# D-Robotics/hobot_stereonet

Measured on AMD Instinct MI355X. Metric: stereo pairs/s at 1280x720 D=192 (ms/frame alongside), higher is better.
Workload: dtype f16 (refinement-tower MFMA operands fp16 — 3x3 weights rounded per kernel so that every kernel's tap sum survives —, LeakyReLU applied after the fp16 rounding; low-resolution branch on 22-bit hi/lo split fp16 operands, 3 fp16 MFMAs per product in every 32-channel layer — profiles/r04_lowres_ablation

## Files before the change

hobot_stereonet_amd/csrc/sn_dbg_hooks.hpp:

```cpp
#pragma once

namespace {

void host_to_slots(const float* src, int nimg, int H, int W, std::vector<_Float16>& dst) {
  const size_t plane = (size_t)H * W;
  dst.assign((size_t)nimg * 8 * plane * 8, (_Float16)0.f);
  for (int img = 0; img < nimg; ++img)
    for (int c = 0; c < kC; ++c)
      for (size_t i = 0; i < plane; ++i) {
        const float v = src[((size_t)img * kC + c) * plane + i];
        const _Float16 hi = (_Float16)v;
        const size_t base = (((size_t)img * 4 + (c >> 3)) * 2) * plane;
        dst[(base + i) * 8 + (c & 7)] = hi;
        dst[(base + plane + i) * 8 + (c & 7)] = (_Float16)((v - (float)hi) * kSplitScale);
      }
}
void host_from_slots(const std::vector<_Float16>& src, int nimg, int H, int W, float* dst) {
  const size_t plane = (size_t)H * W;
  for (int img = 0; img < nimg; ++img)
    for (int c = 0; c < kC; ++c)
      for (size_t i = 0; i < plane; ++i) {
        const size_t base = (((size_t)img * 4 + (c >> 3)) * 2) * plane;
        dst[((size_t)img * kC + c) * plane + i] =
            (float)src[(base + i) * 8 + (c & 7)] + (float)src[(base + plane + i) * 8 + (c & 7)] * kSplitInv;
// ... 236 lines not shown
  for (size_t i = 0; i < be.size(); ++i) beff[i] = (float)be[i];
  return SN_OK;
}

int sn_dbg_down01(sn_handle* h, const int8_t* in6, int h_px, int w, const float* w0, const float* b0, const float* w1,
                  const float* b1, float* out) {
  DevScope ds;
  if (!h || !in6 || !w0 || !b0 || !w1 || !b1 || !out || h_px <= 0 || w <= 0) return SN_ERR_ARG;
  int rc = check_device(h);
  if (rc) return rc;
  const int Hp = (h_px + 15) / 16 * 16, Wp = (w + 15) / 16 * 16, Ho = Hp / 4, Wo = Wp / 4;
  Down01W L;
  rc = upload_down01(h, HostLayer{w0, b0, kC, 3, 25}, HostLayer{w1, b1, kC, kC, 25}, &L);
  ds.adopt(L);
  if (rc) return rc;
  int8_t* din = nullptr;
  uint4* dout = nullptr;
  const size_t nin = (size_t)6 * h_px * w, nout = (size_t)2 * kC * Ho * Wo;
  HIP_TRY(h, ds.alloc(&din, nin));
  HIP_TRY(h, ds.alloc(&dout, nout / 4));
  HIP_TRY(h, hipMemcpy(din, in6, nin, hipMemcpyHostToDevice));
  HIP_TRY(h, launch_down01(h->stream, L, din, h_px, w, 2, Ho, Wo, dout, SlotGeom{Ho, Wo, 0, 0}, h->num_cu));
  HIP_TRY(h, hipStreamSynchronize(h->stream));
  std::vector<_Float16> hs(nout * 2);
  HIP_TRY(h, from_dev(hs, dout));
  host_from_slots(hs, 2, Ho, Wo, out);
  return SN_OK;
}

int sn_dbg_refin(sn_handle* h, const float* disp_low, const int8_t* in6, int h_px, int w, int dmax, const float* wt,
                 const float* bias, int split, float* out) {
  DevScope ds;
  if (!h || !disp_low || !in6 || !wt || !bias || !out || h_px <= 0 || w <= 0 || dmax <= 0) return SN_ERR_ARG;
  int rc = check_device(h);
  if (rc) return rc;
  const int Hp = (h_px + 15) / 16 * 16, Wp = (w + 15) / 16 * 16, hl = Hp / 16, wl = Wp / 16;
  RefHost t(make_ref_geom(Hp, Wp), 1, Hp, Wp, true, true);
  Down0F16 L;
  rc = upload_refin_f16(h, HostLayer{wt, bias, kC, 4, 9}, &L);
  ds.adopt(L);
  if (rc) return rc;
  float *ddl = nullptr, *dbias = nullptr;
  int8_t* din = nullptr;
  uint4* dout = nullptr;
  HIP_TRY(h, ds.alloc(&ddl, (size_t)hl * wl));
  HIP_TRY(h, ds.alloc(&dbias, kC));
  HIP_TRY(h, ds.alloc(&din, (size_t)6 * h_px * w));
  HIP_TRY(h, ds.alloc(&dout, t.slots()));
  HIP_TRY(h, hipMemcpy(ddl, disp_low, (size_t)hl * wl * 4, hipMemcpyHostToDevice));
  HIP_TRY(h, hipMemcpy(dbias, bias, kC * 4, hipMemcpyHostToDevice));
  HIP_TRY(h, hipMemcpy(din, in6, (size_t)6 * h_px * w, hipMemcpyHostToDevice));
  HIP_TRY(h, memset_now(dout, 0, t.slots() * 16));
  HIP_TRY(h, launch_refin_f16(h->stream, L, dbias, ddl, din, false, hl, wl, h_px, w, 1.0f / (float)dmax,
                              UpScale{1.0f / 16.0f, 16.0f}, t.g, 1, dout, split != 0, t.lo_slots * 16, h->num_cu));
  HIP_TRY(h, hipStreamSynchronize(h->stream));
  HIP_TRY(h, from_dev(t.v, dout));
  t.unpack(out, split != 0);
  if (!t.border_is_zero(1)) {
    set_err(h, "ref.in wrote into the zero border");
    return SN_ERR_DEVICE;
  }
  return SN_OK;
}

int sn_dbg_conv3d(sn_handle* h, const float* in, int d, int h_px, int w, const float* wt, const float* bias,
                  int lrelu, float* out) {
  DevScope ds;
  if (!h || !in || !wt || !bias || !out || d <= 0) return SN_ERR_ARG;
  int rc = check_device(h);
  if (rc) return rc;
  const bool x3 = (lrelu & 2) != 0, slots = (lrelu & 4) != 0, dma = (lrelu & 8) != 0;
  lrelu &= 1;
  if (slots != x3 || (dma && !slots)) return SN_ERR_ARG;
  ConvLayer L;
  rc = upload_conv3d(h, HostLayer{wt, bias, kC, kC, 27}, &L);
  if (!rc && x3)
    rc = upload_x3(h, 96, [&](int co, int c, int tap) { return wt[(((size_t)co * kC + (c & 31)) * 3 + (c >> 5)) * 9 + tap]; }, &L);
  ds.adopt(L);
  if (rc) return rc;
  const size_t plane = (size_t)h_px * w, n = (size_t)kC * d * plane;
  std::vector<float> tmp(n);
  for (int ci = 0; ci < kC; ++ci)
    for (int z = 0; z < d; ++z)
      memcpy(&tmp[((size_t)z * kC + ci) * plane], &in[((size_t)ci * d + z) * plane], plane * 4);
  float *din = nullptr, *dout = nullptr;
  HIP_TRY(h, ds.alloc(&din, n));
  HIP_TRY(h, ds.alloc(&dout, n));
  if (slots) {
    std::vector<_Float16> hs, ho(n * 2);
    host_to_slots(tmp.data(), d, h_px, w, hs);
    if (dma) {
      const VolPad g = vol_pad(d, h_px, w);
      PaddedSlots pin(SlotGeom{g.PH, g.PW, 1, 1}, h_px, w, (size_t)d * 8, 8), pout = pin;
      pin.put(hs);
      uint4 *pdin = nullptr, *pdout = nullptr;
      HIP_TRY(h, ds.alloc(&pdin, pin.v.size() / 8));
      HIP_TRY(h, ds.alloc(&pdout, pout.v.size() / 8));
      HIP_TRY(h, to_dev(pdin, pin.v));
      HIP_TRY(h, memset_now(pdout, 0, pout.v.size() * 2));
      HIP_TRY(h, launch_agg_dma<true>(h->stream, L, pdin, g, 1, pdout, lrelu != 0, h->num_cu));
      HIP_TRY(h, hipStreamSynchronize(h->stream));
      HIP_TRY(h, from_dev(pout.v, pdout));
      pout.get(ho);
      if (!pout.outside_is_zero()) {
        set_err(h, "k_agg_x3s_dma wrote outside the image");
        return SN_ERR_DEVICE;
      }
// ... 294 lines not shown
```

hobot_stereonet_amd/csrc/sn_engine.hpp:

```cpp
#pragma once

namespace {

using namespace sn;

constexpr int kNDown = 4, kNFeatRes = 6, kNAgg = 4, kNRefRes = 6;
constexpr int kRefDil[kNRefRes] = {1, 2, 4, 8, 1, 1};
constexpr float kOutScale = 2.60443857769133e-6f;
constexpr double kWireFactor = 16.0 * 12.0;
constexpr double kAutoEnvelopeSingle = 1.0, kAutoEnvelopeMulti = 2.9;
constexpr double kAutoResidualCap = 1e30;
constexpr int kMaxPieceEvents = 64;
constexpr int kMaxTowerStreams = 2;

#define HIP_TRY(h, expr)                                                              \
  do {                                                                                \
    hipError_t e_ = (expr);                                                           \
    if (e_ != hipSuccess) {                                                           \
      set_err(h, std::string(#expr) + ": " + hipGetErrorString(e_));                  \
      return SN_ERR_DEVICE;                                                           \
    }                                                                                 \
  } while (0)

inline hipError_t memset_now(void* p, int v, size_t bytes) {
// ... 123 lines not shown
  hipStream_t stream = nullptr;
  hipEvent_t ev0 = nullptr, ev1 = nullptr;
  Workspace ws;
  int8_t* pin_in = nullptr;
  int32_t* pin_raw = nullptr;
  float* pin_disp = nullptr;
  int32_t* user_raw = nullptr;
  float* user_disp = nullptr;
  uint64_t ticket = 0;
  hipGraphExec_t gexec[2][4][4] = {};
  int uses[2][4][4] = {};
  int mode_run = 0;
};

struct RangeCount {
  unsigned long long level[4] = {}, low = 0;
  bool any() const { return (level[0] | level[1] | level[2] | level[3] | low) != 0; }
};

struct AutoCtl {
  sn_auto_state st{};
  bool calibrated = false;
  bool pending = false;
  int pending_mode = 0, pending_n = 0;
  double selfcheck_epe = -1.0, selfcheck_res = -1.0;
  double last_level[4] = {}, last_res = 0.0;
  RangeCount last_range;
  int last_mode = 0;
  uint64_t calls = 0, pairs = 0, reruns = 0;
};

}

struct sn_handle {
  int device = 0;
  int W = 0, H = 0, D = 0, Wp = 0, Hp = 0, wl = 0, hl = 0, Dl = 0;
  int max_batch = 1, precision = SN_PREC_F16, task_num = 4, refine_chunk = 1, piece = 16;
  AutoCtl actl;
  std::mutex mu_cal;
  float* chk[2] = {nullptr, nullptr};
  hipEvent_t ev_stats = nullptr;
  int refine_chunk_x3 = 1;
  hipStream_t stream = nullptr;
  hipStream_t s_low = nullptr, s_tow[kMaxTowerStreams] = {};
  hipEvent_t ev_fork = nullptr, ev_join = nullptr, ev_tow_join[kMaxTowerStreams] = {}, ev_piece[kMaxPieceEvents] = {};
  bool overlap = true;
  int tower_streams = kMaxTowerStreams;
#if SN_DIAGNOSTICS
  unsigned ablate_x = 0;
#else
  static constexpr unsigned ablate_x = 0;
#endif
  bool obstacle_rle = true;
  bool tail_fuse = true;
  int fuse_mode = 4;
  unsigned* dump = nullptr;
  bool use_graphs = true;
  bool stream_prio = false;
  ConvLayer down[kNDown], fres[kNFeatRes][2], fout, agg[kNAgg];
  Down0F16 down0;
  Down01W down01;
  bool fold_down01 = false;
  HeadLayer aout;
  int levels = 1;
  Tower tw[kMaxLevels];
  int num_cu = 256;
  Workspace ws;
  std::vector<Slot> slots;
  std::mutex mu;
  std::condition_variable cv;
  uint64_t next_ticket = 1;
  bool profiling = false;
  hipEvent_t ev[8] = {};
  hipEvent_t ev_dom[2 * 6] = {};
  int dom_pairs = 0;
  float stage_ms[SN_STAGE_COUNT] = {};
  mutable std::string err;
  mutable std::mutex err_mu;
  struct PointCloudSlots {
    enum { kScratch = 0, kRaw, kNv12, kPoints, kCounts, kPinRaw, kPinNv12, kCount };
  };
  struct PointCloud : Lane<PointCloudSlots> {
    PointCloud() { buf[kPinRaw].pinned = buf[kPinNv12].pinned = true; }
  } pc;
  struct FilterSlots {
    enum { kScratch = 0, kRaw, kDisp, kMask, kCounts, kCount };
  };
  using Filter = Lane<FilterSlots>;
  Filter flt;
  struct SmoothSlots {
    enum { kScratch = 0, kRaw, kGuide, kOut, kDisp, kMask, kCounts, kCount };
  };
  using Smooth = Lane<SmoothSlots>;
  Smooth smo;
  struct JpegSlots {
    enum { kCoef = 0, kBytes, kLens, kIn, kOut, kSizes, kCount };
  };
  struct Jpeg : Lane<JpegSlots> {
    sn::JpgPlan plan;
  } jpg;
  struct RenderSlots {
    enum { kRaw = 0, kLeft, kOut, kCanvas, kCoef, kBytes, kLens, kJpegOut, kSizes, kCount };
  };
  struct Render : Lane<RenderSlots> {
    sn::JpgPlan plan;
  } rnd;
// ... 82 lines not shown
```

hobot_stereonet_amd/csrc/sn_forward.hpp:

```cpp
#pragma once

namespace {

inline int piece_pairs(const sn_handle* h, int nb, int rb) {
  int pb = h->piece > 0 ? h->piece : 16;
  if (pb > nb) pb = nb;
  if (pb < rb) pb = rb;
  return pb;
}
inline int level_chunk_pairs(int rb, int pb, int lv) {
  const long r = (long)rb << (2 * lv);
  return lv == 0 ? rb : (r < pb ? (int)r : pb);
}

int alloc_ws(sn_handle* h, Workspace* ws, int nb, int rb, int ns, int rb_x3 = 0) {
  const bool is_auto = h->precision == SN_PREC_AUTO;
  if (rb_x3 <= 0 || rb_x3 > rb) rb_x3 = rb;
  ws->nb = nb;
  ws->rb = rb;
  ws->rb_x3 = rb_x3;
  ws->ns = (ns > 1 && nb > rb) ? (ns < kMaxTowerStreams ? ns : kMaxTowerStreams) : 1;
  if (h->levels > 1) ws->ns = 1;
  ws->pb = piece_pairs(h, nb, rb);
  const int pb = ws->pb;
// ... 290 lines not shown
  float dnorm;
  float* od;
  int32_t* orw;
  unsigned* chunk_ctr;
  int c;
  int cap;
  bool pe;
  int mode;
  unsigned long long* stat;
};

int refine_level(sn_handle* h, Workspace& ws, hipStream_t st, const RefineCall& a) {
  const Tower& T = *a.T;
  const int ncu = h->num_cu, c = a.c;
  const int tcu = ws.tower_cu > 0 ? ws.tower_cu : ncu;
  const int Hk = T.Hk, Wk = T.Wk;
  const bool pe = a.pe;
  const float inv_q = (float)(1.0 / (kWireFactor * (double)kOutScale));
  if (a.mode == SN_PREC_FP32) {
    LoadRefineIn ld{a.src, reinterpret_cast<const int8_t*>(a.img_src), a.sh, a.sw, a.H, a.W, Hk, Wk, 1.0f / a.dnorm, a.ups,
                    a.pyr ? reinterpret_cast<const float*>(a.img_src) : nullptr};
    if (Hk * Wk <= 64 * 128)
      HIP_TRY(h, (launch_conv<3, 1, 1, 4, 4, 32>(st, T.rin, ld, c, Hk, Wk, a.ref[0], nullptr, true)));
    else
      HIP_TRY(h, (launch_conv<3, 1, 1, 4, 8, 64>(st, T.rin, ld, c, Hk, Wk, a.ref[0], nullptr, true)));
    if (pe) HIP_TRY(h, hipEventRecord(h->ev[4], st));
    for (int i = 0; i < kNRefRes; ++i) {
      HIP_TRY(h, conv3x3(st, T.rres[i][0], a.ref[0], c, Hk, Wk, kRefDil[i], a.ref[1], nullptr, true, ncu));
      HIP_TRY(h, conv3x3(st, T.rres[i][1], a.ref[1], c, Hk, Wk, kRefDil[i], a.ref[0], a.ref[0], true, ncu));
    }
    if (pe) HIP_TRY(h, hipEventRecord(h->ev[5], st));
    const HeadArgs ha{T.rout.w, a.src, a.od, a.orw, T.rout.bias, a.dnorm, inv_q, a.sh, a.sw, a.H, a.W, a.ups, a.stat};
    if (switches().head_mfma32) {
      constexpr int TH = 14;
      using HT = HeadTile<TH>;
      const int tiles_x = (a.W + HT::TWO - 1) / HT::TWO, tiles_y = (a.H + TH - 1) / TH;
      hipLaunchKernelGGL(k_head_final_mfma32<TH>, dim3((unsigned)(tiles_x * tiles_y * c)), dim3(256), HT::LDS_BYTES, st, a.ref[0],
                         Hk, Wk, tiles_x, tiles_y, ha);
    } else {
      dim3 grid((a.W + 63) / 64, (a.H + 3) / 4, c);
      hipLaunchKernelGGL(k_head_final, grid, dim3(256), 0, st, a.ref[0], Hk, Wk, ha);
    }
  } else {
    uint4 *x16 = a.ref16[0], *t16 = a.ref16[1];
    if (pe) h->dom_pairs = 0;
    const bool rev_env = switches().rev;
    RefGeom g = T.rg;
    int launch_no = 0;
    auto flip = [&]() { g.rev = rev_env ? (launch_no++ & 1) : 0; };
    flip();
    const bool x3 = a.mode == SN_PREC_F16X3;
    const size_t lo_slots = ref16_slots(g, a.cap) + ref_slack(g);
    HIP_TRY(h, launch_refin_f16(st, T.refin, T.rin.bias, a.src, a.img_src, a.pyr, a.sh, a.sw, a.H, a.W, 1.0f / a.dnorm, a.ups, g,
                                c, x16, x3, lo_slots * 16, ncu));
    if (pe) HIP_TRY(h, hipEventRecord(h->ev[4], st));
    flip();
    const HeadArgs ha{T.rout.wsplit, a.src, a.od, a.orw, T.rout.biassplit, a.dnorm * T.rout.unscale, inv_q, a.sh, a.sw,
                      a.H, a.W, a.ups, a.stat};
    const bool last_streamed = h->fuse_mode == 4 && stream_block_supports(kRefDil[kNRefRes - 1]);
    const bool tail = !x3 && last_streamed && h->tail_fuse && kRefDil[kNRefRes - 1] == 1 && a.ups.rs <= 0.5f;
    for (int i = 0; i < kNRefRes; ++i) {
      if (x3) {
        const bool dom = pe && stream_x3_supports(kRefDil[i]) && h->dom_pairs < 6;
        if (dom) HIP_TRY(h, hipEventRecord(h->ev_dom[2 * h->dom_pairs], st));
        HIP_TRY(h, ref_block_f16x3(st, T.rres16x3[i][0], T.rres16x3[i][1], g, tcu, kRefDil[i], &x16, &t16, lo_slots, c));
        if (dom) HIP_TRY(h, hipEventRecord(h->ev_dom[2 * h->dom_pairs++ + 1], st));
      } else if (tail && i == kNRefRes - 1) {
        if (pe) HIP_TRY(h, hipEventRecord(h->ev[5], st));
        HIP_TRY(h, ref_block_stream_tail(st, T.rres16[i][0], T.rres16[i][1], g, tcu, x16, c, h->dump, ha));
      } else {
        const bool dom = pe && h->fuse_mode == 4 && stream_block_supports(kRefDil[i]) && h->dom_pairs < 6;
        if (dom) HIP_TRY(h, hipEventRecord(h->ev_dom[2 * h->dom_pairs], st));
        HIP_TRY(h, ref_block_f16(st, T.rres16[i][0], T.rres16[i][1], g, tcu, kRefDil[i], &x16, &t16, c,
                                 a.chunk_ctr + 2 * i * kTileCtrStride, h->fuse_mode, h->dump, rev_env));
        if (dom) HIP_TRY(h, hipEventRecord(h->ev_dom[2 * h->dom_pairs++ + 1], st));
      }
    }
    if (!tail) {
      if (pe) HIP_TRY(h, hipEventRecord(h->ev[5], st));
      HIP_TRY(h, launch_head_final_f16(st, x3, x16, lo_slots, g, c, ha));
    }
  }
  HIP_TRY(h, hipGetLastError());
  return SN_OK;
}

inline int chunk_pairs(const sn_handle* h, const Workspace& ws, int mode, int lv = 0) {
  return (h->precision == SN_PREC_AUTO && mode == SN_PREC_F16X3) ? ws.rbk_x3[lv] : ws.rbk[lv];
}

inline int take_ctr_block(sn_handle* h, Workspace& ws, int* ctr_block, unsigned** out) {
  *out = nullptr;
  if (!ws.tile_ctr) return SN_OK;
  if (*ctr_block >= ws.n_chunks) {
    set_err(h, "internal: tile-queue pool exhausted");
    return SN_ERR_DEVICE;
  }
  *out = ws.tile_ctr + (size_t)(*ctr_block)++ * (kTileCtrBytes / sizeof(unsigned));
  return SN_OK;
}

int refine_coarse(sn_handle* h, Workspace& ws, hipStream_t st, int p0, int m, const int8_t* in6, int* ctr_block, int mode) {
  const size_t HW = (size_t)h->H * h->W;
  const int8_t* in_piece = in6 + (size_t)p0 * 6 * HW;
  for (int lv = 1; lv < h->levels; ++lv) {
    const Tower& T = h->tw[lv];
    const long total = (long)m * 3 * T.Hk * T.Wk;
// ... 342 lines not shown
```

hobot_stereonet_amd/csrc/sn_kernels.hpp:

```cpp
#pragma once
#include <hip/hip_runtime.h>
#include <stdint.h>

#include <type_traits>

#ifndef SN_X3S_FPK
#define SN_X3S_FPK 2
#endif
#ifndef SN_X3S_WAGPR
#define SN_X3S_WAGPR 1
#endif

namespace sn {

typedef float f32x16 __attribute__((ext_vector_type(16)));
typedef float f32x4 __attribute__((ext_vector_type(4)));

typedef _Float16 half8 __attribute__((ext_vector_type(8)));
typedef _Float16 half4 __attribute__((ext_vector_type(4)));

constexpr int kC = 32;
constexpr int kRefPad = 8;
constexpr float kSplitScale = 2048.0f;
constexpr float kSplitInv = 1.0f / 2048.0f;
// ... 1561 lines not shown
#pragma unroll
      for (int i = 0; i < 2 * T::NSTORE; ++i) asm volatile("" : "+v"(rres[i]));
    }
    const bool interior = y0 + T::TH <= g.H && x0 + T::TW <= g.W;
#pragma unroll
    for (int q = 0; q < 4; ++q) {
      char* oq = reinterpret_cast<char*>(out) + (tb + (unsigned)q * plane_b);
      char* oql = out_lo + (tb + (unsigned)q * plane_b);
#pragma unroll
      for (int s = 0; s < T::SPW; ++s) {
        half4 hh, hl;
#pragma unroll
        for (int e = 0; e < 4; ++e) {
          float v = acc0[s][4 * q + e] + acc1[s][4 * q + e] * kSplitInv;
          if (RES) {
            const uint2 rh = rres[RES ? 2 * (s * 4 + q) : 0], rl = rres[RES ? 2 * (s * 4 + q) + 1 : 0];
            const half4 vh = *reinterpret_cast<const half4*>(&rh);
            const half4 vl = *reinterpret_cast<const half4*>(&rl);
            v += (float)vh[e] + (float)vl[e] * kSplitInv;
          }
          if (lrelu) v = lrelu_fast(v);
          const _Float16 hi = (_Float16)v;
          hh[e] = hi;
          hl[e] = (_Float16)((v - (float)hi) * kSplitScale);
        }
        if (!interior) {
          const int seg = seg0 + s;
          const int y = y0 + seg / T::CSEG, x = x0 + (seg % T::CSEG) * 32 + j;
          if (!(y < g.H && x < g.W)) {
            hh = half4{(_Float16)0.f, (_Float16)0.f, (_Float16)0.f, (_Float16)0.f};
            hl = hh;
          }
        }
        *reinterpret_cast<half4*>(oq + io_voff[s]) = hh;
        *reinterpret_cast<half4*>(oql + io_voff[s]) = hl;
      }
    }
    img = nimg_;
    y0 = ny0;
    x0 = nx0;
  }
}

template <int TW_>
struct RefInTile {
  static constexpr int TH = 8, TW = TW_, CSEG = TW / 32;
  static constexpr int ROWS = TH + 2, COLS = TW + 8;
  static constexpr int BUF = ROWS * COLS;
  static constexpr int LDS_BYTES = 2 * BUF * 16;
  static constexpr int NUNIT = ROWS * (COLS / 4);
  static constexpr int SPW = TH * CSEG / 4;
};

template <bool SPLIT, bool PYR, int TW>
__global__ __launch_bounds__(256, 2) void k_refin_f16(const float* __restrict__ disp_low,
                                                   const void* __restrict__ img_src,
                                                   int hl, int wl, int H, int W, float inv_d, UpScale ups,
                                                   const uint4* __restrict__ wfrag,
                                                   const float* __restrict__ bias, uint4* __restrict__ out,
                                                   size_t lo_off_bytes, RefGeom g, int nimg, int al4) {
  using T = RefInTile<TW>;
  static_assert(T::NUNIT <= 256, "one staging unit per thread");
  extern __shared__ __attribute__((aligned(16))) uint4 s_px[];
  const int tid = threadIdx.x, lane = tid & 63;
  const int wave = __builtin_amdgcn_readfirstlane(tid >> 6);
  const int j = lane & 31, gk = lane >> 5;

  half8 wa[5], wb[5];
#pragma unroll
  for (int t = 0; t < 5; ++t) {
    const uint4 a = wfrag[(2 * t) * 64 + lane], b = wfrag[(2 * t + 1) * 64 + lane];
    wa[t] = *reinterpret_cast<const half8*>(&a);
    wb[t] = *reinterpret_cast<const half8*>(&b);
  }
  f32x16 bv;
#pragma unroll
  for (int r = 0; r < 16; ++r) bv[r] = bias[(r & 3) + 8 * (r >> 2) + 4 * gk];
  int koff[5];
#pragma unroll
  for (int t = 0; t < 5; ++t) {
    int tap = 2 * t + gk;
    tap = tap < 9 ? tap : 0;
    koff[t] = (tap / 3) * T::COLS + (tap % 3) + 3;
  }

  const int per_img = g.tiles_x * g.tiles_y;
  const int total = per_img * nimg;
  const int ur = tid / (T::COLS / 4), uq = tid - ur * (T::COLS / 4);
  const bool unit = tid < T::NUNIT;
  const int8_t* const in6 = reinterpret_cast<const int8_t*>(img_src);
  const float* const pyr = reinterpret_cast<const float*>(img_src);
  const bool x16 = ups.rs == 1.0f / 16.0f;
  uint32_t pimg[3];
  float pf[PYR ? 3 : 1][4];
  float pd[4];
  bool pval[4];
  auto fetch = [&](int tile) {
    if (g.rev) tile = total - 1 - tile;
    const int img = tile / per_img, rem = tile - img * per_img;
    const int ty = rem / g.tiles_x, tx = rem - ty * g.tiles_x;
    const int y = ty * T::TH - 1 + ur, x = tx * T::TW - 4 + 4 * uq;
    pimg[0] = pimg[1] = pimg[2] = 0;
#pragma unroll
    for (int k = 0; k < 4; ++k) {
      pd[k] = 0.f;
      pval[k] = false;
    }
    if (!unit || (unsigned)y >= (unsigned)g.H) return;
    const float* dl = disp_low + (size_t)img * hl * wl;
#pragma unroll
    for (int k = 0; k < 4; ++k) pval[k] = (unsigned)(x + k) < (unsigned)g.W;
    if (x16 && x >= 0) {
      float sy = ((float)y + 0.5f) * ups.rs - 0.5f;
      sy = sy < 0.f ? 0.f : sy;
      float sx0 = ((float)x + 0.5f) * ups.rs - 0.5f;
// ... 23 lines not shown
        for (int k = 0; k < 4; ++k) pf[PYR ? c : 0][k] = pval[k] ? row[x + k] : 0.f;
      }
    } else if (y < H) {
#pragma unroll
      for (int c = 0; c < 3; ++c) {
        const int8_t* row = in6 + (((size_t)img * 6 + c) * H + y) * (size_t)W;
        uint32_t v = 0;
        if (al4) {
          if (x >= 0 && x + 3 < W) v = *reinterpret_cast<const uint32_t*>(row + x);
        } else {
#pragma unroll
          for (int k = 0; k < 4; ++k)
            if ((unsigned)(x + k) < (unsigned)W) v |= (uint32_t)(uint8_t)row[x + k] << (8 * k);
        }
        pimg[c] = v;
      }
    }
  };
  auto commit = [&](uint4* buf) {
    if (!unit) return;
#pragma unroll
    for (int k = 0; k < 4; ++k) {
      half8 sl;
#pragma unroll
      for (int e = 0; e < 8; ++e) sl[e] = (_Float16)0.f;
      if (pval[k]) {
        const _Float16 dh = (_Float16)pd[k];
        sl[0] = dh;
        sl[4] = (_Float16)((pd[k] - (float)dh) * kSplitScale);
        if (PYR) {
#pragma unroll
          for (int c = 0; c < 3; ++c) {
            const float v = pf[PYR ? c : 0][k];
            const _Float16 vh = (_Float16)v;
            sl[1 + c] = vh;
            sl[5 + c] = (_Float16)((v - (float)vh) * kSplitScale);
          }
        } else {
#pragma unroll
          for (int c = 0; c < 3; ++c) sl[1 + c] = (_Float16)((float)(int8_t)(pimg[c] >> (8 * k)) * (1.0f / 128.0f));
        }
      }
      buf[ur * T::COLS + 4 * uq + k] = *reinterpret_cast<const uint4*>(&sl);
    }
  };

  int tile = blockIdx.x;
  if (tile >= total) return;
  fetch(tile);
  commit(s_px);
  __syncthreads();
  int cur = 0;
  const unsigned plane_b = (unsigned)g.Hs * (unsigned)g.Ws * 16u;
  unsigned io_voff[T::SPW];
#pragma unroll
  for (int s = 0; s < T::SPW; ++s) {
    const int seg = wave * T::SPW + s;
    io_voff[s] = ((unsigned)(seg / T::CSEG) * (unsigned)g.Ws + (unsigned)((seg % T::CSEG) * 32 + j)) * 16u + gk * 8u;
  }
  for (; tile < total; tile += gridDim.x) {
    const int nxt = tile + gridDim.x;
    if (nxt < total) fetch(nxt);
    const uint4* buf = s_px + cur * T::BUF;
    f32x16 acc0[T::SPW], acc1[T::SPW];
    f32x16 zero;
#pragma unroll
    for (int r = 0; r < 16; ++r) zero[r] = 0.f;
#pragma unroll
    for (int t = 0; t < 5; ++t) {
#pragma unroll
      for (int s = 0; s < T::SPW; ++s) {
        const int seg = wave * T::SPW + s;
        const int srow = seg / T::CSEG, scol = (seg % T::CSEG) * 32;
        const uint4 xv = buf[koff[t] + srow * T::COLS + scol + j];
        const half8 xb = *reinterpret_cast<const half8*>(&xv);
        acc0[s] = __builtin_amdgcn_mfma_f32_32x32x16_f16(wa[t], xb, t == 0 ? bv : acc0[s], 0, 0, 0);
        acc1[s] = __builtin_amdgcn_mfma_f32_32x32x16_f16(wb[t], xb, t == 0 ? zero : acc1[s], 0, 0, 0);
      }
    }
    {
      const int tile_m = g.rev ? total - 1 - tile : tile;
      const int img = tile_m / per_img, rem = tile_m - img * per_img;
      const int ty = rem / g.tiles_x, tx = rem - ty * g.tiles_x;
      const int y0 = ty * T::TH, x0 = tx * T::TW;
      const bool interior = y0 + T::TH <= g.H && x0 + T::TW <= g.W;
      const unsigned tb = (((unsigned)img * 4u * (unsigned)g.Hs + (unsigned)(y0 + kRefPad)) * (unsigned)g.Ws +
                           (unsigned)(x0 + kRefPad)) * 16u;
#pragma unroll
      for (int s = 0; s < T::SPW; ++s) {
#pragma unroll
        for (int q = 0; q < 4; ++q) {
          char* oq = reinterpret_cast<char*>(out) + (tb + (unsigned)q * plane_b);
          char* oql = oq + lo_off_bytes;
          half4 hh, hl4;
          if (SPLIT) {
#pragma unroll
            for (int e = 0; e < 4; ++e) {
              float v = acc0[s][4 * q + e] + acc1[s][4 * q + e] * kSplitInv;
              v = lrelu_fast(v);
              const _Float16 hi = (_Float16)v;
              hh[e] = hi;
              hl4[e] = (_Float16)((v - (float)hi) * kSplitScale);
            }
          } else {
            float v[4];
#pragma unroll
            for (int e = 0; e < 4; ++e) v[e] = acc0[s][4 * q + e] + acc1[s][4 * q + e] * kSplitInv;
            const uint2 pk{act_pack2_f16(v[0], v[1], (_Float16)kSlope), act_pack2_f16(v[2], v[3], (_Float16)kSlope)};
            hh = *reinterpret_cast<const half4*>(&pk);
          }
          bool ok = true;
          if (!interior) {
            const int seg = wave * T::SPW + s;
            ok = y0 + seg / T::CSEG < g.H && x0 + (seg % T::CSEG) * 32 + j < g.W;
          }
          if (ok) {
            *reinterpret_cast<half4*>(oq + io_voff[s]) = hh;
            if (SPLIT) *reinterpret_cast<half4*>(oql + io_voff[s]) = hl4;
          }
        }
      }
    }
    if (nxt < total) commit(s_px + (cur ^ 1) * T::BUF);
    lds_barrier();
    cur ^= 1;
  }
}

template <int TH_>
struct HeadTile {
  static constexpr int TH = TH_, TWO = 62;
  static constexpr int RP = TH + 2, CP = 64;
  static constexpr int NSEG = RP * 2, SPW = (NSEG + 3) / 4;
  static constexpr int PLANE = RP * CP;
  static constexpr int LDS_BYTES = 9 * PLANE * 4;
};

template <int TH>
__device__ __forceinline__ void head_window_finish(const float* s_p, int n, int y0, int x0, const HeadArgs& ha) {
  using T = HeadTile<TH>;
  const float* dl = ha.disp_low + (size_t)n * ha.hl * ha.wl;
  float moved = 0.f;
  unsigned bad = 0u;
  for (int p = threadIdx.x; p < T::TH * T::TWO; p += 256) {
    const int oy = p / T::TWO, ox = p - oy * T::TWO;
    const int y = y0 + oy, x = x0 + ox;
    if (y >= ha.H || x >= ha.W) continue;
    float acc = ha.bias;
#pragma unroll
    for (int ky = 0; ky < 3; ++ky)
#pragma unroll
      for (int kx = 0; kx < 3; ++kx) acc += s_p[(ky * 3 + kx) * T::PLANE + (oy + ky) * T::CP + ox + kx];
    float mv;
    unsigned nf;
    const float d = head_value(upsample_map(dl, ha.hl, ha.wl, y, x, ha.ups), ha.dmax, acc, mv, nf);
    moved += mv;
    bad += nf;
    head_store(ha.out_disp, ha.out_raw, ((size_t)n * ha.H + y) * ha.W + x, d, ha.inv_q);
  }
  refine_stat_commit_block(ha.stat, moved, bad);
}

template <bool SPLIT, int TH>
__global__ __launch_bounds__(256) void k_head_final_f16(const uint4* __restrict__ xin, size_t lo_slots, RefGeom g,
                                                        int tiles_x, int tiles_y, HeadArgs ha) {
  using T = HeadTile<TH>;
  extern __shared__ __attribute__((aligned(16))) float s_p[];
  const int tid = threadIdx.x, lane = tid & 63;
  const int wave = __builtin_amdgcn_readfirstlane(tid >> 6);
  const int j = lane & 31, gh = lane >> 5;
  int t = blockIdx.x;
  const int tx = t % tiles_x;
  t /= tiles_x;
  const int ty = t % tiles_y, n = t / tiles_y;
  const int y0 = ty * T::TH, x0 = tx * T::TWO;

// ... 118 lines not shown
```

hobot_stereonet_amd/csrc/sn_launch.hpp:

```cpp
#pragma once

namespace {

template <class K>
hipError_t ensure_lds_attr(K kern, int bytes) {
  static std::mutex mu;
  static std::unordered_map<const void*, unsigned long long> done;
  int dev = 0;
  if (hipGetDevice(&dev) != hipSuccess) dev = 0;
  const unsigned long long bit = 1ull << (dev & 63);
  const void* key = reinterpret_cast<const void*>(kern);
  std::lock_guard<std::mutex> lk(mu);
  unsigned long long& m = done[key];
  if (m & bit) return hipSuccess;
  const hipError_t e = hipFuncSetAttribute(key, hipFuncAttributeMaxDynamicSharedMemorySize, bytes);
  if (e == hipSuccess) m |= bit;
  return e;
}

inline ConvArgs make_conv_args(const ConvLayer& L, const void* w, void* out, const void* res, int nimg, int Ho, int Wo, int dil,
                               int pad, bool lrelu, int TR, int TC) {
  ConvArgs a{};
  a.wpk = reinterpret_cast<const float*>(w);
  a.bias = L.bias;
  a.out = reinterpret_cast<float*>(out);
  a.res = reinterpret_cast<const float*>(res);
  a.nimg = nimg;
  a.cin_pad = L.cin_pad;
  a.Ho = Ho;
  a.Wo = Wo;
  a.dil = dil;
  a.pad = pad;
  a.lrelu = lrelu ? 1 : 0;
  a.tiles_x = (Wo + TC - 1) / TC;
  a.tiles_y = (Ho + TR - 1) / TR;
  return a;
}

inline int xcd_band_grid(int cap, int total) {
  const int need = (total + 7) / 8 * 8;
  return ((cap > need ? need : cap) + 7) / 8 * 8;
}

template <int TW>
hipError_t launch_refin_f16_tw(hipStream_t st, const Down0F16& L, const float* bias, const float* disp_low,
                               const void* img_src, bool pyr, int hl, int wl, int H, int W, float inv_d, UpScale ups,
                               RefGeom g, int nimg, uint4* out, bool split, size_t lo_off_bytes, int num_cu) {
  using T = RefInTile<TW>;
  g.tiles_x = (g.W + TW - 1) / TW;
  g.tiles_y = (g.H + T::TH - 1) / T::TH;
  const int total = g.tiles_x * g.tiles_y * nimg;
  int blocks = 2 * num_cu;
  if (blocks > total) blocks = total;
  const int al4 = !pyr && (W % 4 == 0) && (reinterpret_cast<uintptr_t>(img_src) % 4 == 0);
#define SN_REFIN(S, P)                                                                                             \
  hipLaunchKernelGGL((k_refin_f16<S, P, TW>), dim3(blocks), dim3(256), T::LDS_BYTES, st, disp_low, img_src, hl, wl, H, \
                     W, inv_d, ups, L.wfrag, bias, out, lo_off_bytes, g, nimg, al4)
  if (split && pyr) SN_REFIN(true, true);
  else if (split) SN_REFIN(true, false);
  else if (pyr) SN_REFIN(false, true);
  else SN_REFIN(false, false);
#undef SN_REFIN
  return hipGetLastError();
}

hipError_t launch_refin_f16(hipStream_t st, const Down0F16& L, const float* bias, const float* disp_low,
                            const void* img_src, bool pyr, int hl, int wl, int H, int W, float inv_d, UpScale ups,
                            const RefGeom& g, int nimg, uint4* out, bool split, size_t lo_off_bytes, int num_cu) {
  return launch_refin_f16_tw<64>(st, L, bias, disp_low, img_src, pyr, hl, wl, H, W, inv_d, ups, g, nimg, out, split,
                                 lo_off_bytes, num_cu);
}

hipError_t launch_down0_f16(hipStream_t st, const Down0F16& L, const float* bias, const int8_t* in6, int H, int W,
                            int nimg, int Ho, int Wo, float* out, int num_cu, const SlotGeom* og = nullptr) {
  constexpr int TC = 32;
  using T = Down0Tile<TC>;
  const int tiles_x = (Wo + TC - 1) / TC, tiles_y = (Ho + T::TR - 1) / T::TR;
  const int total = tiles_x * tiles_y * nimg;
  int blocks = 2 * num_cu;
  if (blocks > total) blocks = total;
  const int al4 = (W % 4 == 0) && (reinterpret_cast<uintptr_t>(in6) % 4 == 0);
  hipLaunchKernelGGL((k_down0_f16<TC>), dim3(blocks), dim3(256), T::LDS_BYTES, st, in6, H, W, L.wfrag, bias, out, Ho, Wo,
                     tiles_x, tiles_y, nimg, 0, al4, og ? og->PH : Ho, og ? og->PW : Wo, og ? og->py : 0, og ? og->px : 0);
  return hipGetLastError();
}

template <bool W4>
hipError_t launch_down01_w(hipStream_t st, const Down01W& L, const int8_t* in6, int H, int W, int nimg, int Ho, int Wo,
                           uint4* out, const SlotGeom& og, int num_cu) {
  using T = Down01;
  hipError_t e = ensure_lds_attr(k_down01_f16<W4>, T::LDS_BYTES);
  if (e != hipSuccess) return e;
  const int tiles_x = (Wo + T::TC - 1) / T::TC, tiles_y = (Ho + T::TR - 1) / T::TR;
  const int total = tiles_x * tiles_y * nimg;
  int blocks = num_cu / 8 * 8;
  while (blocks > 8 && blocks / 8 > (total + 7) / 8) blocks -= 8;
  hipLaunchKernelGGL(k_down01_f16<W4>, dim3(blocks), dim3(256), T::LDS_BYTES, st, in6, H, W,
                     L.wfrag + (size_t)T::INNER * T::NK * 2 * 64, L.bias + T::INNER * kC, out, Ho, Wo, tiles_x, tiles_y, nimg,
                     og.PH, og.PW, og.py, og.px);
  const int per_img = 4 + 2 * ((Wo - 2 + 31) / 32) + 2 * ((Ho - 2 + 31) / 32);
  hipLaunchKernelGGL(k_down01_border<W4>, dim3(per_img * (nimg / 2)), dim3(192), 0, st, in6, H, W, L.wfrag, L.bias, out,
                     Ho, Wo, nimg, og.PH, og.PW, og.py, og.px);
  return hipGetLastError();
}
hipError_t launch_down01(hipStream_t st, const Down01W& L, const int8_t* in6, int H, int W, int nimg, int Ho, int Wo,
                         uint4* out, const SlotGeom& og, int num_cu) {
  return (W % 4) == 0 ? launch_down01_w<true>(st, L, in6, H, W, nimg, Ho, Wo, out, og, num_cu)
                      : launch_down01_w<false>(st, L, in6, H, W, nimg, Ho, Wo, out, og, num_cu);
}

template <int KS, int STRIDE, int VCH, int TR, int TC, int SEGW, int MINB, bool OUTSLOT, class Loader, bool HASRES = false>
hipError_t launch_conv_x3s(hipStream_t st, const ConvLayer& L, const Loader& ld, int nimg, int Ho, int Wo, float* out,
                           const float* res, bool lrelu, int num_cu) {
  using T = X3sTile<KS, STRIDE, VCH, TR, TC, SEGW>;
  const ConvArgs a = make_conv_args(L, L.wx3, out, res, nimg, Ho, Wo, 1, KS / 2, lrelu, TR, TC);
  if (res != nullptr && !HASRES)
    return launch_conv_x3s<KS, STRIDE, VCH, TR, TC, SEGW, MINB, OUTSLOT, Loader, true>(st, L, ld, nimg, Ho, Wo, out, res, lrelu, num_cu);
  auto kern = k_conv_x3s<KS, STRIDE, VCH, TR, TC, SEGW, MINB, OUTSLOT, HASRES, Loader>;
  static_assert(T::LDS_BYTES <= 160 * 1024, "x3s tile does not fit the LDS");
  if (T::LDS_BYTES > 64 * 1024) {
    hipError_t e = ensure_lds_attr(kern, (int)T::LDS_BYTES);
    if (e != hipSuccess) return e;
  }
// ... 384 lines not shown
```

hobot_stereonet_amd/csrc/sn_switches.hpp:

```cpp
#pragma once

#include <cctype>
#include <climits>
#include <cstdlib>
#include <cstring>
#include <string>

#include "../../include/stereonet_hip.h"

#ifndef SN_DIAGNOSTICS
#define SN_DIAGNOSTICS 0
#endif

namespace sn {

constexpr int kSwitchUnset = INT_MIN;

enum { kAblDown = 0, kAblFeat = 3, kAblAgg = 16, kAblCount = 20 };

struct Switches {
  bool down01 = true;
  bool agg_dma = true;
  bool feat_dma = true;
  bool down_dma = true;
  bool head_fold = true;
  int f32_grid = 0;
  bool f32_tower = true;
  int stream_wgs = 0;
  int stream_dil = 8;
  int fuse = 4;
  bool x3_stream = true;
  int x3_nwr = 4;
  int first_piece = 0;
  bool head_mfma32 = true;
  bool rev = true;
  bool async_share = true;

  bool w_round_sum_preserving = true;
  int precision = SN_PREC_AUTO;
  int tower_streams = kSwitchUnset;
  int stream_priority = kSwitchUnset;
  bool no_overlap = false;
  bool no_graph = false;
  bool tail_fuse = true;
  bool obstacle_rle = true;
  int mgpu_gather = 0;
  bool mgpu_allow_dup = false;
  unsigned ablate_w = 0;
  unsigned ablate_x = 0;
};

namespace switch_parse {
inline bool on_unless_zero(const char* name) {
  const char* e = getenv(name);
  return !(e != nullptr && atoi(e) == 0);
}
inline bool present(const char* name) { return getenv(name) != nullptr; }
inline int int_or(const char* name, int dflt) {
  const char* e = getenv(name);
  return e ? atoi(e) : dflt;
}
inline bool equals(const char* name, const char* value) {
  const char* e = getenv(name);
  return e && strcmp(e, value) == 0;
}

#if !SN_DIAGNOSTICS
inline unsigned ablate_mask(const char*) { return 0u; }
#else
inline unsigned ablate_mask(const char* var) {
  const char* e = getenv(var);
  if (!e || !*e) return 0u;
  if (!strcmp(e, "all")) return (1u << kAblCount) - 1u;
  unsigned m = 0;
  std::string str(e);
  size_t pos = 0;
  while (pos <= str.size()) {
    size_t c = str.find(',', pos);
    if (c == std::string::npos) c = str.size();
    const std::string t = str.substr(pos, c - pos);
    int idx = -1;
    if (t.rfind("down", 0) == 0 && t.size() == 5 && t[4] >= '1' && t[4] <= '3') idx = kAblDown + (t[4] - '1');
    else if (t.rfind("agg", 0) == 0 && t.size() == 4 && t[3] >= '0' && t[3] <= '3') idx = kAblAgg + (t[3] - '0');
    else if (t.size() >= 2 && t[0] == 'f' && atoi(t.c_str() + 1) >= 0 && atoi(t.c_str() + 1) <= 12 && isdigit((unsigned char)t[1])) idx = kAblFeat + atoi(t.c_str() + 1);
    if (idx >= 0) m |= 1u << idx;
    pos = c + 1;
  }
  return m;
}
#endif
}

inline void read_switches(Switches* s, bool process_scope) {
  using namespace switch_parse;
  if (process_scope) {
    const bool plain = ablate_mask("SN_ABLATE_X") != 0;
    s->down01 = on_unless_zero("SN_DOWN01");
    s->agg_dma = on_unless_zero("SN_AGG_DMA") && !plain;
    s->feat_dma = on_unless_zero("SN_FEAT_DMA") && !plain;
    s->down_dma = on_unless_zero("SN_DOWN_DMA") && !plain;
    s->head_fold = on_unless_zero("SN_HEAD_FOLD");
    s->f32_grid = int_or("SN_F32_GRID", 0);
    s->f32_tower = on_unless_zero("SN_F32_TOWER");
    s->stream_wgs = int_or("SN_STREAM_WGS", 0);
    s->stream_dil = int_or("SN_STREAM_DIL", 8);
    s->fuse = int_or("SN_FUSE", 4);
    s->x3_stream = on_unless_zero("SN_X3_STREAM");
    s->x3_nwr = int_or("SN_X3_NWR", 4);
    s->first_piece = int_or("SN_FIRST_PIECE", 0);
    s->head_mfma32 = on_unless_zero("SN_HEAD_MFMA32");
    s->rev = on_unless_zero("SN_REV");
    s->async_share = on_unless_zero("SN_ASYNC_SHARE");
    return;
  }
  s->w_round_sum_preserving = !equals("SN_W_ROUND", "rne");
  s->precision = equals("SN_PRECISION", "f16") ? SN_PREC_F16 : equals("SN_PRECISION", "f16x3") ? SN_PREC_F16X3
                 : equals("SN_PRECISION", "fp32") ? SN_PREC_FP32 : SN_PREC_AUTO;
  s->tower_streams = int_or("SN_TOWER_STREAMS", kSwitchUnset);
  s->stream_priority = equals("SN_STREAM_PRIORITY", "") ? kSwitchUnset : int_or("SN_STREAM_PRIORITY", kSwitchUnset);
  s->no_overlap = present("SN_NO_OVERLAP");
  s->no_graph = present("SN_NO_GRAPH");
  s->tail_fuse = on_unless_zero("SN_TAIL_FUSE");
  s->obstacle_rle = on_unless_zero("SN_OBSTACLE_RLE");
  s->mgpu_gather = equals("SN_MGPU_GATHER", "peer") ? 1 : equals("SN_MGPU_GATHER", "rccl") ? 2 : 0;
  s->mgpu_allow_dup = int_or("SN_MGPU_ALLOW_DUP", 0) == 1;
  s->ablate_w = ablate_mask("SN_ABLATE_W");
  s->ablate_x = ablate_mask("SN_ABLATE_X");
}

inline const Switches& switches() {
  static const Switches latched = [] {
    Switches s;
    read_switches(&s, true);
    return s;
  }();
  return latched;
}
inline Switches switches_at_create() {
  Switches s = switches();
  read_switches(&s, false);
  return s;
}

}
```

hobot_stereonet_amd/csrc/stereonet_hip.hip:

```cpp
#include <hip/hip_runtime.h>

#include <algorithm>

#include <atomic>
#include <chrono>
#include <cmath>
#include <condition_variable>
#include <cstdio>
#include <cstdlib>
#include <cstring>
#include <memory>
#include <mutex>
#include <string>
#include <unordered_map>
#include <vector>

#include "../../include/stereonet_hip.h"
#include "sn_internal.h"
#include "sn_switches.hpp"
#include "sn_kernels.hpp"
#include "sn_pointcloud.hpp"
#include "sn_lrcheck.hpp"
#include "sn_dispfilter.hpp"
#include "sn_confidence.hpp"
// ... 158 lines not shown
    const double low_elems = 2.0 * pb * kC * (h->Hp / 2.0) * (h->Wp / 2.0);
    const double vol_elems = (double)pb * h->Dl * kC * h->hl * h->wl;
    double ref_bytes = 0;
    for (int lv = 0; lv < h->levels; ++lv) {
      const RefGeom& rg = h->tw[lv].rg;
      const double b = ((double)level_chunk_pairs(h->refine_chunk, pb, lv) * 4.0 * rg.Hs * rg.Ws + (double)ref_slack(rg) + (double)ref_front(rg)) * 16.0;
      if (b > ref_bytes) ref_bytes = b;
    }
    if (low_elems >= 4.0e9 || ref_bytes >= 4.0e9 || vol_elems >= 4.0e9) {
      delete h;
      return SN_ERR_ARG;
    }
  }
  int rc = check_device(h);
  auto fail = [&](int code) {
    create_fail(code, h->err.empty() ? "engine set-up" : h->err.c_str());
    sn_destroy(h);
    return code;
  };
  if (rc) return fail(rc);
  if (hipStreamCreateWithFlags(&h->stream, hipStreamNonBlocking) != hipSuccess) return fail(SN_ERR_DEVICE);
  for (auto& e : h->ev)
    if (hipEventCreate(&e) != hipSuccess) return fail(SN_ERR_DEVICE);
  for (auto& e : h->ev_dom)
    if (hipEventCreate(&e) != hipSuccess) return fail(SN_ERR_DEVICE);
  if (hipEventCreateWithFlags(&h->ev_stats, hipEventDisableTiming) != hipSuccess) return fail(SN_ERR_DEVICE);
  if (c.precision == SN_PREC_AUTO)
    for (auto& p : h->chk)
      if (dalloc(&p, (size_t)H * W) != hipSuccess) return fail(SN_ERR_NOMEM);
  int prio = 0;
  {
    int least = 0, greatest = 0;
    const bool want = sw.stream_priority != kSwitchUnset ? sw.stream_priority == 1 : stream_prio == 1;
    if (want && hipDeviceGetStreamPriorityRange(&least, &greatest) == hipSuccess) prio = greatest;
  }
  h->stream_prio = prio != 0;
  auto mk_stream = [&](hipStream_t* st) {
    return prio != 0 ? hipStreamCreateWithPriority(st, hipStreamNonBlocking, prio) : hipStreamCreateWithFlags(st, hipStreamNonBlocking);
  };
  if (mk_stream(&h->s_low) != hipSuccess ||
      hipEventCreateWithFlags(&h->ev_fork, hipEventDisableTiming) != hipSuccess ||
      hipEventCreateWithFlags(&h->ev_join, hipEventDisableTiming) != hipSuccess)
    return fail(SN_ERR_DEVICE);
  for (int i = 0; i < kMaxTowerStreams; ++i)
    if (mk_stream(&h->s_tow[i]) != hipSuccess ||
        hipEventCreateWithFlags(&h->ev_tow_join[i], hipEventDisableTiming) != hipSuccess)
      return fail(SN_ERR_DEVICE);
  for (auto& e : h->ev_piece)
    if (hipEventCreateWithFlags(&e, hipEventDisableTiming) != hipSuccess) return fail(SN_ERR_DEVICE);
  h->overlap = !sw.no_overlap;
  h->use_graphs = !sw.no_graph;
  h->fuse_mode = sw.fuse;
  h->tail_fuse = sw.tail_fuse;
  h->obstacle_rle = sw.obstacle_rle;
  if (hipMalloc(reinterpret_cast<void**>(&h->dump), 4096) != hipSuccess) return fail(SN_ERR_NOMEM);

  BlobWalker bw{blob.data()};
  const bool low_x3 = h->precision != SN_PREC_FP32;
  const unsigned abl_w = sw.ablate_w;
#if SN_DIAGNOSTICS
  h->ablate_x = sw.ablate_x;
#endif
  int feat_idx = 0;
  h->fold_down01 = low_x3 && sw.down01;
  HostLayer hl_down0{};
  for (int i = 0; i < kNDown; ++i) {
    const HostLayer hl_ = bw.next(kC, i == 0 ? 3 : kC, 25);
    if ((rc = upload_conv2d(h, hl_, 4, &h->down[i]))) return fail(rc);
    if (low_x3 && i == 0 && (rc = upload_down0_f16(h, hl_, &h->down0))) return fail(rc);
    if (i == 0) hl_down0 = hl_;
    if (h->fold_down01 && i == 1 && (rc = upload_down01(h, hl_down0, hl_, &h->down01))) return fail(rc);
    if (low_x3 && i > 0 &&
        (rc = upload_x3(h, kC, [&](int co, int c, int tap) { return hl_.w[((size_t)co * kC + c) * 25 + tap]; },
                        &h->down[i], 25, (abl_w >> (kAblDown + i - 1)) & 1u)))
      return fail(rc);
  }
  auto up2d = [&](ConvLayer* L) -> int {
    const HostLayer hl_ = bw.next(kC, kC, 9);
    int r = upload_conv2d(h, hl_, 8, L);
    if (r || !low_x3) return r;
    const bool z = (abl_w >> (kAblFeat + feat_idx)) & 1u;
    ++feat_idx;
    return upload_x3(h, kC, [&](int co, int c, int tap) { return hl_.w[((size_t)co * kC + c) * 9 + tap]; }, L, 9, z);
  };
  for (int i = 0; i < kNFeatRes; ++i)
    for (int j = 0; j < 2; ++j)
      if ((rc = up2d(&h->fres[i][j]))) return fail(rc);
  if ((rc = up2d(&h->fout))) return fail(rc);
  for (int i = 0; i < kNAgg; ++i) {
    const HostLayer hl_ = bw.next(kC, kC, 27);
    if ((rc = upload_conv3d(h, hl_, &h->agg[i]))) return fail(rc);
    if (low_x3 && (rc = upload_x3(h, 96, [&](int co, int c, int tap) {
          return hl_.w[(((size_t)co * kC + (c & 31)) * 3 + (c >> 5)) * 9 + tap];
        }, &h->agg[i], 9, (abl_w >> (kAblAgg + i)) & 1u)))
      return fail(rc);
  }
  {
    const HostLayer hl_ = bw.next(1, kC, 27);
    if ((rc = upload_head(h, hl_, &h->aout))) return fail(rc);
    if (low_x3 && (rc = upload_agg_head_frag(h, hl_, &h->aout))) return fail(rc);
  }
  for (int lv = 0; lv < h->levels; ++lv) {
    Tower& T = h->tw[lv];
    {
      const HostLayer hl_ = bw.next(kC, 4, 9);
      if ((rc = upload_conv2d(h, hl_, 4, &T.rin))) return fail(rc);
// ... 566 lines not shown
```

Measured before the change: 3100.

## Process refin segments in passes to cut accumulators and raise occupancy

The refinement-input kernel now computes its per-wave segments one pass at a time instead of keeping accumulators for all segments live, and drops the per-segment precomputed output offsets. This cuts VGPR pressure, so the launch bounds and grid go from 2 to 4 blocks per CU when multi-pass is on. In the pyramid path the next-tile fetch is moved after compute so its staging registers don't overlap the accumulators, at the cost of less prefetch overlap. The behaviour is on by default and SN_REFIN_PASS=0 turns it off.

```diff
diff --git a/hobot_stereonet_amd/csrc/sn_dbg_hooks.hpp b/hobot_stereonet_amd/csrc/sn_dbg_hooks.hpp
--- a/hobot_stereonet_amd/csrc/sn_dbg_hooks.hpp
+++ b/hobot_stereonet_amd/csrc/sn_dbg_hooks.hpp
@@ -312,7 +312,8 @@
   HIP_TRY(h, hipMemcpy(din, in6, (size_t)6 * h_px * w, hipMemcpyHostToDevice));
   HIP_TRY(h, memset_now(dout, 0, t.slots() * 16));
   HIP_TRY(h, launch_refin_f16(h->stream, L, dbias, ddl, din, false, hl, wl, h_px, w, 1.0f / (float)dmax,
-                              UpScale{1.0f / 16.0f, 16.0f}, t.g, 1, dout, split != 0, t.lo_slots * 16, h->num_cu));
+                              UpScale{1.0f / 16.0f, 16.0f}, t.g, 1, dout, split != 0, t.lo_slots * 16, h->num_cu,
+                              h->refin_pass));
   HIP_TRY(h, hipStreamSynchronize(h->stream));
   HIP_TRY(h, from_dev(t.v, dout));
   t.unpack(out, split != 0);
diff --git a/hobot_stereonet_amd/csrc/sn_engine.hpp b/hobot_stereonet_amd/csrc/sn_engine.hpp
--- a/hobot_stereonet_amd/csrc/sn_engine.hpp
+++ b/hobot_stereonet_amd/csrc/sn_engine.hpp
@@ -199,6 +199,7 @@
   static constexpr unsigned ablate_x = 0;
 #endif
   bool obstacle_rle = true;
+  bool refin_pass = true;
   bool tail_fuse = true;
   int fuse_mode = 4;
   unsigned* dump = nullptr;
diff --git a/hobot_stereonet_amd/csrc/sn_forward.hpp b/hobot_stereonet_amd/csrc/sn_forward.hpp
--- a/hobot_stereonet_amd/csrc/sn_forward.hpp
+++ b/hobot_stereonet_amd/csrc/sn_forward.hpp
@@ -366,7 +366,7 @@
     const bool x3 = a.mode == SN_PREC_F16X3;
     const size_t lo_slots = ref16_slots(g, a.cap) + ref_slack(g);
     HIP_TRY(h, launch_refin_f16(st, T.refin, T.rin.bias, a.src, a.img_src, a.pyr, a.sh, a.sw, a.H, a.W, 1.0f / a.dnorm, a.ups, g,
-                                c, x16, x3, lo_slots * 16, ncu));
+                                c, x16, x3, lo_slots * 16, ncu, h->refin_pass));
     if (pe) HIP_TRY(h, hipEventRecord(h->ev[4], st));
     flip();
     const HeadArgs ha{T.rout.wsplit, a.src, a.od, a.orw, T.rout.biassplit, a.dnorm * T.rout.unscale, inv_q, a.sh, a.sw,
diff --git a/hobot_stereonet_amd/csrc/sn_kernels.hpp b/hobot_stereonet_amd/csrc/sn_kernels.hpp
--- a/hobot_stereonet_amd/csrc/sn_kernels.hpp
+++ b/hobot_stereonet_amd/csrc/sn_kernels.hpp
@@ -1637,8 +1637,8 @@
   static constexpr int SPW = TH * CSEG / 4;
 };
 
-template <bool SPLIT, bool PYR, int TW>
-__global__ __launch_bounds__(256, 2) void k_refin_f16(const float* __restrict__ disp_low,
+template <bool SPLIT, bool PYR, int TW, int PASS>
+__global__ __launch_bounds__(256, PASS >= RefInTile<TW>::SPW ? 2 : 4) void k_refin_f16(const float* __restrict__ disp_low,
                                                    const void* __restrict__ img_src,
                                                    int hl, int wl, int H, int W, float inv_d, UpScale ups,
                                                    const uint4* __restrict__ wfrag,
@@ -1646,6 +1646,8 @@
                                                    size_t lo_off_bytes, RefGeom g, int nimg, int al4) {
   using T = RefInTile<TW>;
   static_assert(T::NUNIT <= 256, "one staging unit per thread");
+  constexpr int NP = PASS < T::SPW ? PASS : T::SPW;
+  static_assert(T::SPW % NP == 0, "whole passes");
   extern __shared__ __attribute__((aligned(16))) uint4 s_px[];
   const int tid = threadIdx.x, lane = tid & 63;
   const int wave = __builtin_amdgcn_readfirstlane(tid >> 6);
@@ -1775,45 +1777,44 @@
   __syncthreads();
   int cur = 0;
   const unsigned plane_b = (unsigned)g.Hs * (unsigned)g.Ws * 16u;
-  unsigned io_voff[T::SPW];
-#pragma unroll
-  for (int s = 0; s < T::SPW; ++s) {
-    const int seg = wave * T::SPW + s;
-    io_voff[s] = ((unsigned)(seg / T::CSEG) * (unsigned)g.Ws + (unsigned)((seg % T::CSEG) * 32 + j)) * 16u + gk * 8u;
-  }
+  const unsigned io_voff = (unsigned)j * 16u + gk * 8u;
   for (; tile < total; tile += gridDim.x) {
     const int nxt = tile + gridDim.x;
-    if (nxt < total) fetch(nxt);
+    constexpr bool LATE_FETCH = PYR && NP < T::SPW;
+    if (!LATE_FETCH && nxt < total) fetch(nxt);
     const uint4* buf = s_px + cur * T::BUF;
-    f32x16 acc0[T::SPW], acc1[T::SPW];
-    f32x16 zero;
-#pragma unroll
-    for (int r = 0; r < 16; ++r) zero[r] = 0.f;
-#pragma unroll
-    for (int t = 0; t < 5; ++t) {
-#pragma unroll
-      for (int s = 0; s < T::SPW; ++s) {
-        const int seg = wave * T::SPW + s;
-        const int srow = seg / T::CSEG, scol = (seg % T::CSEG) * 32;
-        const uint4 xv = buf[koff[t] + srow * T::COLS + scol + j];
-        const half8 xb = *reinterpret_cast<const half8*>(&xv);
-        acc0[s] = __builtin_amdgcn_mfma_f32_32x32x16_f16(wa[t], xb, t == 0 ? bv : acc0[s], 0, 0, 0);
-        acc1[s] = __builtin_amdgcn_mfma_f32_32x32x16_f16(wb[t], xb, t == 0 ? zero : acc1[s], 0, 0, 0);
-      }
-    }
-    {
-      const int tile_m = g.rev ? total - 1 - tile : tile;
-      const int img = tile_m / per_img, rem = tile_m - img * per_img;
-      const int ty = rem / g.tiles_x, tx = rem - ty * g.tiles_x;
-      const int y0 = ty * T::TH, x0 = tx * T::TW;
-      const bool interior = y0 + T::TH <= g.H && x0 + T::TW <= g.W;
-      const unsigned tb = (((unsigned)img * 4u * (unsigned)g.Hs + (unsigned)(y0 + kRefPad)) * (unsigned)g.Ws +
-                           (unsigned)(x0 + kRefPad)) * 16u;
-#pragma unroll
-      for (int s = 0; s < T::SPW; ++s) {
+    const int tile_m = g.rev ? total - 1 - tile : tile;
+    const int img = tile_m / per_img, rem = tile_m - img * per_img;
+    const int ty = rem / g.tiles_x, tx = rem - ty * g.tiles_x;
+    const int y0 = ty * T::TH, x0 = tx * T::TW;
+    const bool interior = y0 + T::TH <= g.H && x0 + T::TW <= g.W;
+    const unsigned tb = (((unsigned)img * 4u * (unsigned)g.Hs + (unsigned)(y0 + kRefPad)) * (unsigned)g.Ws +
+                         (unsigned)(x0 + kRefPad)) * 16u;
+#pragma unroll
+    for (int s0 = 0; s0 < T::SPW; s0 += NP) {
+      f32x16 acc0[NP], acc1[NP];
+      f32x16 zero;
+#pragma unroll
+      for (int r = 0; r < 16; ++r) zero[r] = 0.f;
+#pragma unroll
+      for (int t = 0; t < 5; ++t) {
+#pragma unroll
+        for (int s = 0; s < NP; ++s) {
+          const int seg = wave * T::SPW + s0 + s;
+          const int srow = seg / T::CSEG, scol = (seg % T::CSEG) * 32;
+          const uint4 xv = buf[koff[t] + srow * T::COLS + scol + j];
+          const half8 xb = *reinterpret_cast<const half8*>(&xv);
+          acc0[s] = __builtin_amdgcn_mfma_f32_32x32x16_f16(wa[t], xb, t == 0 ? bv : acc0[s], 0, 0, 0);
+          acc1[s] = __builtin_amdgcn_mfma_f32_32x32x16_f16(wb[t], xb, t == 0 ? zero : acc1[s], 0, 0, 0);
+        }
+      }
+#pragma unroll
+      for (int s = 0; s < NP; ++s) {
 #pragma unroll
         for (int q = 0; q < 4; ++q) {
-          char* oq = reinterpret_cast<char*>(out) + (tb + (unsigned)q * plane_b);
+          const int seg = wave * T::SPW + s0 + s;
+          const unsigned sb = ((unsigned)(seg / T::CSEG) * (unsigned)g.Ws + (unsigned)((seg % T::CSEG) * 32)) * 16u;
+          char* oq = reinterpret_cast<char*>(out) + (tb + sb + (unsigned)q * plane_b);
           char* oql = oq + lo_off_bytes;
           half4 hh, hl4;
           if (SPLIT) {
@@ -1834,17 +1835,19 @@
           }
           bool ok = true;
           if (!interior) {
-            const int seg = wave * T::SPW + s;
             ok = y0 + seg / T::CSEG < g.H && x0 + (seg % T::CSEG) * 32 + j < g.W;
           }
           if (ok) {
-            *reinterpret_cast<half4*>(oq + io_voff[s]) = hh;
-            if (SPLIT) *reinterpret_cast<half4*>(oql + io_voff[s]) = hl4;
+            *reinterpret_cast<half4*>(oq + io_voff) = hh;
+            if (SPLIT) *reinterpret_cast<half4*>(oql + io_voff) = hl4;
           }
         }
       }
     }
-    if (nxt < total) commit(s_px + (cur ^ 1) * T::BUF);
+    if (nxt < total) {
+      if (LATE_FETCH) fetch(nxt);
+      commit(s_px + (cur ^ 1) * T::BUF);
+    }
     lds_barrier();
     cur ^= 1;
   }
diff --git a/hobot_stereonet_amd/csrc/sn_launch.hpp b/hobot_stereonet_amd/csrc/sn_launch.hpp
--- a/hobot_stereonet_amd/csrc/sn_launch.hpp
+++ b/hobot_stereonet_amd/csrc/sn_launch.hpp
@@ -42,7 +42,7 @@
   return ((cap > need ? need : cap) + 7) / 8 * 8;
 }
 
-template <int TW>
+template <int TW, int PASS>
 hipError_t launch_refin_f16_tw(hipStream_t st, const Down0F16& L, const float* bias, const float* disp_low,
                                const void* img_src, bool pyr, int hl, int wl, int H, int W, float inv_d, UpScale ups,
                                RefGeom g, int nimg, uint4* out, bool split, size_t lo_off_bytes, int num_cu) {
@@ -50,11 +50,11 @@
   g.tiles_x = (g.W + TW - 1) / TW;
   g.tiles_y = (g.H + T::TH - 1) / T::TH;
   const int total = g.tiles_x * g.tiles_y * nimg;
-  int blocks = 2 * num_cu;
+  int blocks = (PASS < T::SPW ? 4 : 2) * num_cu;
   if (blocks > total) blocks = total;
   const int al4 = !pyr && (W % 4 == 0) && (reinterpret_cast<uintptr_t>(img_src) % 4 == 0);
 #define SN_REFIN(S, P)                                                                                             \
-  hipLaunchKernelGGL((k_refin_f16<S, P, TW>), dim3(blocks), dim3(256), T::LDS_BYTES, st, disp_low, img_src, hl, wl, H, \
+  hipLaunchKernelGGL((k_refin_f16<S, P, TW, PASS>), dim3(blocks), dim3(256), T::LDS_BYTES, st, disp_low, img_src, hl, wl, H, \
                      W, inv_d, ups, L.wfrag, bias, out, lo_off_bytes, g, nimg, al4)
   if (split && pyr) SN_REFIN(true, true);
   else if (split) SN_REFIN(true, false);
@@ -66,9 +66,12 @@
 
 hipError_t launch_refin_f16(hipStream_t st, const Down0F16& L, const float* bias, const float* disp_low,
                             const void* img_src, bool pyr, int hl, int wl, int H, int W, float inv_d, UpScale ups,
-                            const RefGeom& g, int nimg, uint4* out, bool split, size_t lo_off_bytes, int num_cu) {
-  return launch_refin_f16_tw<64>(st, L, bias, disp_low, img_src, pyr, hl, wl, H, W, inv_d, ups, g, nimg, out, split,
-                                 lo_off_bytes, num_cu);
+                            const RefGeom& g, int nimg, uint4* out, bool split, size_t lo_off_bytes, int num_cu,
+                            bool pass) {
+  return pass ? launch_refin_f16_tw<64, 1>(st, L, bias, disp_low, img_src, pyr, hl, wl, H, W, inv_d, ups, g, nimg, out,
+                                           split, lo_off_bytes, num_cu)
+              : launch_refin_f16_tw<64, RefInTile<64>::SPW>(st, L, bias, disp_low, img_src, pyr, hl, wl, H, W, inv_d, ups, g,
+                                                            nimg, out, split, lo_off_bytes, num_cu);
 }
 
 hipError_t launch_down0_f16(hipStream_t st, const Down0F16& L, const float* bias, const int8_t* in6, int H, int W,
diff --git a/hobot_stereonet_amd/csrc/sn_switches.hpp b/hobot_stereonet_amd/csrc/sn_switches.hpp
--- a/hobot_stereonet_amd/csrc/sn_switches.hpp
+++ b/hobot_stereonet_amd/csrc/sn_switches.hpp
@@ -43,6 +43,7 @@
   bool no_overlap = false;
   bool no_graph = false;
   bool tail_fuse = true;
+  bool refin_pass = true;
   bool obstacle_rle = true;
   int mgpu_gather = 0;
   bool mgpu_allow_dup = false;
@@ -121,6 +122,7 @@
   s->no_overlap = present("SN_NO_OVERLAP");
   s->no_graph = present("SN_NO_GRAPH");
   s->tail_fuse = on_unless_zero("SN_TAIL_FUSE");
+  s->refin_pass = on_unless_zero("SN_REFIN_PASS");
   s->obstacle_rle = on_unless_zero("SN_OBSTACLE_RLE");
   s->mgpu_gather = equals("SN_MGPU_GATHER", "peer") ? 1 : equals("SN_MGPU_GATHER", "rccl") ? 2 : 0;
   s->mgpu_allow_dup = int_or("SN_MGPU_ALLOW_DUP", 0) == 1;
diff --git a/hobot_stereonet_amd/csrc/stereonet_hip.hip b/hobot_stereonet_amd/csrc/stereonet_hip.hip
--- a/hobot_stereonet_amd/csrc/stereonet_hip.hip
+++ b/hobot_stereonet_amd/csrc/stereonet_hip.hip
@@ -234,6 +234,7 @@
   h->use_graphs = !sw.no_graph;
   h->fuse_mode = sw.fuse;
   h->tail_fuse = sw.tail_fuse;
+  h->refin_pass = sw.refin_pass;
   h->obstacle_rle = sw.obstacle_rle;
   if (hipMalloc(reinterpret_cast<void**>(&h->dump), 4096) != hipSuccess) return fail(SN_ERR_NOMEM);
 
```

After: 3111 (median of 6 runs). About the same (+0.3%).
